# ishine/minimax-speech

Hardware: AMD Instinct MI355X
Metric: 24 kHz audio-seconds generated per wall-second per node (CosyVoice2-0.5B-shaped LM + flow + DAC-VAE, end to end) (higher is better)
Workload: dtype bf16

## Files before the change

### minimax-speech_amd/csrc/attention_x.hip

```cpp
#include "common.h"
#include "../../include/mmx_hip.h"
#include <cstdlib>
#include <type_traits>
#include <utility>

namespace {

__device__ __forceinline__ int swz(int row, int c) { return row * 128 + ((c ^ (row & 7)) << 4); }

__device__ __forceinline__ void split4(const float x[4], uint2& hi, uint2& lo) {
    hi.x = pack_bf16x2(x[0], x[1]);
    hi.y = pack_bf16x2(x[2], x[3]);
    lo.x = pack_bf16x2(x[0] - __uint_as_float(hi.x << 16), x[1] - __uint_as_float(hi.x & 0xffff0000u));
    lo.y = pack_bf16x2(x[2] - __uint_as_float(hi.y << 16), x[3] - __uint_as_float(hi.y & 0xffff0000u));
}

template <int MF, bool PRE, int NW>
__global__ __launch_bounds__(64 * NW) void attn_flash_x_kernel(
    const void* __restrict__ q_, long ldq, long q_bs, const void* __restrict__ k_, long ldk, long k_bs,
    const void* __restrict__ v_, long ldv, long v_bs, float* __restrict__ out, long ldo, long o_bs,
    int Tn, float scale, const float* __restrict__ keymask, long km_bs, int chunk, int nq, int nheads, int npairs,
    int q_begin, const int32_t* __restrict__ klen) {
    typedef std::conditional_t<PRE, bf16_t, float> TI;
    const TI* q = reinterpret_cast<const TI*>(q_);
    const TI* k = reinterpret_cast<const TI*>(k_);
    const TI* v = reinterpret_cast<const TI*>(v_);
    constexpr int D = 64, KT = 64, QW = 16 * MF;
    constexpr int TILE = KT * 128;
    extern __shared__ __attribute__((aligned(16))) char smem[];
    char* Kh = smem;
    char* Kl = Kh + 2 * TILE;
    char* Vh = Kl + 2 * TILE;
    char* Vl = Vh + 2 * TILE;
    char* Ph = Vl + 2 * TILE;
    char* Pl = Ph + NW * QW * 128;
    const int tid = threadIdx.x, lane = tid & 63, wave = tid >> 6;
    const int g = lane >> 4, l16 = lane & 15;
    const int xcd = blockIdx.x & 7, slot = blockIdx.x >> 3;
    const int pair = (slot / nq) * 8 + xcd;
    if (pair >= npairs) return;
    const int qt = slot % nq;
    const int b = pair / nheads, h = pair % nheads;
    const int qb = q_begin + qt * (NW * QW) + wave * QW;
    q += (long)b * q_bs + h * D;
    k += (long)b * k_bs + h * D;
    v += PRE ? (long)b * v_bs + (long)h * D * ldv : (long)b * v_bs + h * D;
    out += (long)b * o_bs + h * D;
    const float* km = keymask ? keymask + (long)b * km_bs : nullptr;
    const float sc2 = scale * 1.44269504088896341f;
    const int Tk = klen ? (klen[b] < Tn ? klen[b] : Tn) : Tn;
    if (klen && q_begin + qt * (NW * QW) >= Tk) {
        for (int id = tid; id < NW * QW * 16; id += 64 * NW) {
            const int i = q_begin + qt * (NW * QW) + (id >> 4);
            if (i < Tn) *reinterpret_cast<float4*>(out + (long)i * ldo + (id & 15) * 4) = make_float4(0.f, 0.f, 0.f, 0.f);
        }
        return;
    }

    short8_t aqh[MF][2], aql[MF][2];
#pragma unroll
    for (int mf = 0; mf < MF; ++mf) {
        int row = qb + mf * 16 + l16;
        row = row < Tn ? row : Tn - 1;
#pragma unroll
        for (int ks = 0; ks < 2; ++ks) {
            if constexpr (PRE) {
                const bf16_t* qp = reinterpret_cast<const bf16_t*>(q) + (long)row * ldq + ks * 32 + 8 * g;
                aqh[mf][ks] = *reinterpret_cast<const short8_t*>(qp);
                aql[mf][ks] = *reinterpret_cast<const short8_t*>(qp + 1024);
            } else {
                const float* qp = reinterpret_cast<const float*>(q) + (long)row * ldq + ks * 32 + 8 * g;
                const float4 a = *reinterpret_cast<const float4*>(qp), c = *reinterpret_cast<const float4*>(qp + 4);
                const float x0[4] = {a.x, a.y, a.z, a.w}, x1[4] = {c.x, c.y, c.z, c.w};
                uint2 h0, l0, h1, l1;
                split4(x0, h0, l0);
                split4(x1, h1, l1);
                aqh[mf][ks] = __builtin_bit_cast(short8_t, make_uint4(h0.x, h0.y, h1.x, h1.y));
                aql[mf][ks] = __builtin_bit_cast(short8_t, make_uint4(l0.x, l0.y, l1.x, l1.y));
            }
        }
    }
    float4_t o[MF][4];
    float m_run[MF], l_run[MF];
    int lim[MF];
#pragma unroll
    for (int mf = 0; mf < MF; ++mf) {
#pragma unroll
        for (int i = 0; i < 4; ++i) o[mf][i] = float4_t{0.f, 0.f, 0.f, 0.f};
        m_run[mf] = -INFINITY;
        l_run[mf] = 0.f;
        const int i = qb + mf * 16 + l16;
        int e = Tk;
        if (chunk > 0) { int c2 = (i / chunk + 1) * chunk; e = c2 < e ? c2 : e; }
        lim[mf] = e;
    }
    int kend = Tk;
    if (chunk > 0) {
        int qlast = q_begin + qt * (NW * QW) + NW * QW - 1;
        if (qlast > Tn - 1) qlast = Tn - 1;
        int e = (qlast / chunk + 1) * chunk;
        if (e < kend) kend = e;
    }
    const int ntile = (kend + KT - 1) / KT;
    int vis_all = Tk;
    if (chunk > 0) {
        const int e = ((q_begin + qt * (NW * QW)) / chunk + 1) * chunk;
        if (e < vis_all) vis_all = e;
    }
    char* Pwh = Ph + wave * QW * 128;
    char* Pwl = Pl + wave * QW * 128;

    constexpr int NT = 64 * NW, CPT = 1024 / NT;
    float4 kreg[CPT], vreg[CPT];
    auto load_tiles = [&](int j0) {
        if constexpr (PRE) {
            const bf16_t* kb = reinterpret_cast<const bf16_t*>(k);
            const bf16_t* vb = reinterpret_cast<const bf16_t*>(v);
#pragma unroll
            for (int pi = 0; pi < CPT / 2; ++pi) {
                const int id = tid + pi * NT, r = id >> 3, c = (id & 7) * 8;
                const int key = j0 + r;
#pragma unroll
                for (int pl = 0; pl < 2; ++pl) {
                    kreg[2 * pi + pl] = key < Tk ? *reinterpret_cast<const float4*>(kb + (long)key * ldk + pl * 1024 + c) : make_float4(0.f, 0.f, 0.f, 0.f);
                    vreg[2 * pi + pl] = (j0 + c < Tk) ? *reinterpret_cast<const float4*>(vb + (long)pl * 512 * ldv + (long)r * ldv + j0 + c) : make_float4(0.f, 0.f, 0.f, 0.f);
                }
            }
            return;
        }
#pragma unroll
        for (int i = 0; i < CPT; ++i) {
            const int id = tid + i * NT;
            const int kr = j0 + (id >> 4);
            kreg[i] = kr < Tk ? *reinterpret_cast<const float4*>(reinterpret_cast<const float*>(k) + (long)kr * ldk + (id & 15) * 4) : make_float4(0.f, 0.f, 0.f, 0.f);
            const int vr = j0 + 2 * (id >> 5) + (id & 1);
            vreg[i] = vr < Tk ? *reinterpret_cast<const float4*>(reinterpret_cast<const float*>(v) + (long)vr * ldv + ((id >> 1) & 15) * 4) : make_float4(0.f, 0.f, 0.f, 0.f);
        }
    };
    auto store_tiles = [&](int buf) {
        if constexpr (PRE) {
#pragma unroll
            for (int pi = 0; pi < CPT / 2; ++pi) {
                const int id = tid + pi * NT, r = id >> 3, c8 = id & 7;
                const int off = buf * TILE + swz(r, c8);
                *reinterpret_cast<float4*>(Kh + off) = kreg[2 * pi];
                *reinterpret_cast<float4*>(Kl + off) = kreg[2 * pi + 1];
                *reinterpret_cast<float4*>(Vh + off) = vreg[2 * pi];
                *reinterpret_cast<float4*>(Vl + off) = vreg[2 * pi + 1];
            }
            return;
        }
#pragma unroll
        for (int i = 0; i < CPT; ++i) {
            const int id = tid + i * NT;
            {
                const int r = id >> 4, c4 = id & 15;
                const float x[4] = {kreg[i].x, kreg[i].y, kreg[i].z, kreg[i].w};
                uint2 hi, lo;
                split4(x, hi, lo);
                const int off = buf * TILE + swz(r, c4 >> 1) + (c4 & 1) * 8;
                *reinterpret_cast<uint2*>(Kh + off) = hi;
                *reinterpret_cast<uint2*>(Kl + off) = lo;
            }
            {
                const int par = id & 1, cc = (id >> 1) & 15, kp = id >> 5;
                const float s0 = par ? vreg[i].x : vreg[i].z, s1 = par ? vreg[i].y : vreg[i].w;
                const float r0 = __shfl_xor(s0, 1, 64), r1 = __shfl_xor(s1, 1, 64);
                const float a0 = par ? r0 : vreg[i].x, b0 = par ? vreg[i].z : r0;
                const float a1 = par ? r1 : vreg[i].y, b1 = par ? vreg[i].w : r1;
                const int d0 = 4 * cc + 2 * par;
                const unsigned h0 = pack_bf16x2(a0, b0), h1 = pack_bf16x2(a1, b1);
                const unsigned l0 = pack_bf16x2(a0 - __uint_as_float(h0 << 16), b0 - __uint_as_float(h0 & 0xffff0000u));
                const unsigned l1 = pack_bf16x2(a1 - __uint_as_float(h1 << 16), b1 - __uint_as_float(h1 & 0xffff0000u));
                const int o0 = buf * TILE + swz(d0, kp >> 2) + (kp & 3) * 4, o1 = buf * TILE + swz(d0 + 1, kp >> 2) + (kp & 3) * 4;
                *reinterpret_cast<unsigned*>(Vh + o0) = h0;
                *reinterpret_cast<unsigned*>(Vl + o0) = l0;
                *reinterpret_cast<unsigned*>(Vh + o1) = h1;
                *reinterpret_cast<unsigned*>(Vl + o1) = l1;
            }
        }
    };
    load_tiles(0);
    store_tiles(0);
    if (ntile > 1) load_tiles(KT);
    for (int jt = 0; jt < ntile; ++jt) {
        const int j0 = jt * KT, buf = jt & 1;
        __syncthreads();
        if (jt + 1 < ntile) store_tiles(buf ^ 1);
        if (jt + 2 < ntile) load_tiles(j0 + 2 * KT);
        float4_t s[MF][4];
#pragma unroll
        for (int nf = 0; nf < 4; ++nf) {
#pragma unroll
            for (int mf = 0; mf < MF; ++mf) s[mf][nf] = float4_t{0.f, 0.f, 0.f, 0.f};
#pragma unroll
            for (int ks = 0; ks < 2; ++ks) {
                const int off = buf * TILE + swz(nf * 16 + l16, ks * 4 + g);
                const short8_t bkh = *reinterpret_cast<const short8_t*>(Kh + off);
                const short8_t bkl = *reinterpret_cast<const short8_t*>(Kl + off);
#pragma unroll
                for (int mf = 0; mf < MF; ++mf) {
                    s[mf][nf] = __builtin_amdgcn_mfma_f32_16x16x32_bf16(bkh, aqh[mf][ks], s[mf][nf], 0, 0, 0);
                    s[mf][nf] = __builtin_amdgcn_mfma_f32_16x16x32_bf16(bkh, aql[mf][ks], s[mf][nf], 0, 0, 0);
                    s[mf][nf] = __builtin_amdgcn_mfma_f32_16x16x32_bf16(bkl, aqh[mf][ks], s[mf][nf], 0, 0, 0);
                }
            }
        }
        const bool need_mask = km || (j0 + KT > vis_all);
        bool kvis[4][4];
        if (need_mask) {
#pragma unroll
            for (int nf = 0; nf < 4; ++nf)
#pragma unroll
                for (int r = 0; r < 4; ++r) {
                    const int j = j0 + nf * 16 + 4 * g + r;
                    kvis[nf][r] = j < Tk && (!km || km[j] != 0.f);
                }
        }
        auto softmax_tile = [&](auto mask_c, auto mf_c) {
            constexpr bool MASK = decltype(mask_c)::value;
            constexpr int mf = decltype(mf_c)::value;
            float mx = -INFINITY;
#pragma unroll
            for (int nf = 0; nf < 4; ++nf)
#pragma unroll
                for (int r = 0; r < 4; ++r) {
                    float x = s[mf][nf][r];
                    if constexpr (MASK) {
                        const int j = j0 + nf * 16 + 4 * g + r;
                        x = (j < lim[mf] && kvis[nf][r]) ? x : -INFINITY;
                        s[mf][nf][r] = x;
                    }
                    mx = fmaxf(mx, x);
                }
            mx *= sc2;
            float m_use = m_run[mf];
            const bool grow = (mx - m_run[mf]) > 6.0f || m_run[mf] == -INFINITY;
            if (__any(grow)) {
                mx = fmaxf(mx, __shfl_xor(mx, 16, 64));
                mx = fmaxf(mx, __shfl_xor(mx, 32, 64));
                const float m_new = fmaxf(m_run[mf], mx);
                const float m_safe = m_new == -INFINITY ? 0.f : m_new;
                const float alpha = __builtin_amdgcn_exp2f(m_run[mf] - m_safe);
                l_run[mf] *= alpha;
#pragma unroll
                for (int df = 0; df < 4; ++df)
#pragma unroll
                    for (int r = 0; r < 4; ++r) o[mf][df][r] *= alpha;
                m_run[mf] = m_new;
                m_use = m_safe;
            }
            float rs = 0.f;
#pragma unroll
            for (int nf = 0; nf < 4; ++nf) {
                float p[4];
#pragma unroll
                for (int r = 0; r < 4; ++r) p[r] = __builtin_amdgcn_exp2f(__builtin_fmaf(s[mf][nf][r], sc2, -m_use));
                rs += (p[0] + p[1]) + (p[2] + p[3]);
                uint2 hi, lo;
                split4(p, hi, lo);
                const int off = swz(mf * 16 + l16, nf * 2 + (g >> 1)) + (g & 1) * 8;
                *reinterpret_cast<uint2*>(Pwh + off) = hi;
                *reinterpret_cast<uint2*>(Pwl + off) = lo;
            }
            l_run[mf] += rs;
        };
        if (need_mask) {
            softmax_tile(std::true_type{}, std::integral_constant<int, 0>{});
            if constexpr (MF > 1) softmax_tile(std::true_type{}, std::integral_constant<int, MF - 1>{});
        } else {
            softmax_tile(std::false_type{}, std::integral_constant<int, 0>{});
            if constexpr (MF > 1) softmax_tile(std::false_type{}, std::integral_constant<int, MF - 1>{});
        }
        __builtin_amdgcn_fence(__ATOMIC_RELEASE, "wavefront");
        __builtin_amdgcn_wave_barrier();
        short8_t aph[MF][2], apl[MF][2];
#pragma unroll
        for (int mf = 0; mf < MF; ++mf)
#pragma unroll
            for (int ks = 0; ks < 2; ++ks) {
                const int off = swz(mf * 16 + l16, ks * 4 + g);
                aph[mf][ks] = *reinterpret_cast<const short8_t*>(Pwh + off);
                apl[mf][ks] = *reinterpret_cast<const short8_t*>(Pwl + off);
            }
#pragma unroll
        for (int df = 0; df < 4; ++df)
#pragma unroll
            for (int ks = 0; ks < 2; ++ks) {
                const int off = buf * TILE + swz(df * 16 + l16, ks * 4 + g);
                const short8_t bvh = *reinterpret_cast<const short8_t*>(Vh + off);
                const short8_t bvl = *reinterpret_cast<const short8_t*>(Vl + off);
#pragma unroll
                for (int mf = 0; mf < MF; ++mf) {
                    o[mf][df] = __builtin_amdgcn_mfma_f32_16x16x32_bf16(bvh, aph[mf][ks], o[mf][df], 0, 0, 0);
                    o[mf][df] = __builtin_amdgcn_mfma_f32_16x16x32_bf16(bvh, apl[mf][ks], o[mf][df], 0, 0, 0);
                    o[mf][df] = __builtin_amdgcn_mfma_f32_16x16x32_bf16(bvl, aph[mf][ks], o[mf][df], 0, 0, 0);
                }
            }
        __builtin_amdgcn_wave_barrier();
    }
#pragma unroll
    for (int mf = 0; mf < MF; ++mf) {
        l_run[mf] += __shfl_xor(l_run[mf], 16, 64);
        l_run[mf] += __shfl_xor(l_run[mf], 32, 64);
    }
#pragma unroll
    for (int mf = 0; mf < MF; ++mf) {
        const int i = qb + mf * 16 + l16;
        if (i >= Tn) continue;
        const float inv = l_run[mf] > 0.f ? 1.f / l_run[mf] : 0.f;
#pragma unroll
        for (int df = 0; df < 4; ++df)
            *reinterpret_cast<float4*>(out + (long)i * ldo + df * 16 + 4 * g) =
                make_float4(o[mf][df][0] * inv, o[mf][df][1] * inv, o[mf][df][2] * inv, o[mf][df][3] * inv);
    }
}

__global__ __launch_bounds__(256) void attn_relpos_x_kernel(
    const float* __restrict__ q, long ldq, long q_bs, const float* __restrict__ k, long ldk, long k_bs,
    const float* __restrict__ v, long ldv, long v_bs, const float* __restrict__ pos, long ldp,
    const float* __restrict__ pos_u, const float* __restrict__ pos_v, float* __restrict__ out, long ldo, long o_bs,
    int Tn, float scale, int chunk, int nq, int nheads, int npairs, const int32_t* __restrict__ klen) {
    constexpr int D = 64, KT = 64, NW = 4, QW = 16, BW = 84;
    constexpr int TILE = KT * 128;
    extern __shared__ __attribute__((aligned(16))) char smem[];
    char* Kh = smem;
    char* Kl = Kh + 2 * TILE;
    char* Vh = Kl + 2 * TILE;
    char* Vl = Vh + 2 * TILE;
    char* Ph = Vl + 2 * TILE;
    char* Pl = Ph + NW * QW * 128;
    float* Bp = reinterpret_cast<float*>(Pl + NW * QW * 128);
    const int tid = threadIdx.x, lane = tid & 63, wave = tid >> 6;
    const int g = lane >> 4, l16 = lane & 15;
    const int xcd = blockIdx.x & 7, slot = blockIdx.x >> 3;
    const int pair = (slot / nq) * 8 + xcd;
    if (pair >= npairs) return;
    const int qt = slot % nq;
    const int b = pair / nheads, h = pair % nheads;
    const int qb = qt * (NW * QW) + wave * QW;
    q += (long)b * q_bs + h * D;
    k += (long)b * k_bs + h * D;
    v += (long)b * v_bs + h * D;
    out += (long)b * o_bs + h * D;
    pos += h * D;
    const float sc2 = scale * 1.44269504088896341f;
    const int Tk = klen ? (klen[b] < Tn ? klen[b] : Tn) : Tn;

    short8_t auh[2], aul[2], avh[2], avl[2];
    {
        int row = qb + l16;
        row = row < Tn ? row : Tn - 1;
#pragma unroll
        for (int ks = 0; ks < 2; ++ks) {
            const float* qp = q + (long)row * ldq + ks * 32 + 8 * g;
            const float4 a = *reinterpret_cast<const float4*>(qp), c = *reinterpret_cast<const float4*>(qp + 4);
            const float* pu = pos_u + h * D + ks * 32 + 8 * g;
            const float* pv = pos_v + h * D + ks * 32 + 8 * g;
            const float x[8] = {a.x, a.y, a.z, a.w, c.x, c.y, c.z, c.w};
            float xu0[4], xu1[4], xv0[4], xv1[4];
#pragma unroll
            for (int e = 0; e < 4; ++e) {
                xu0[e] = x[e] + pu[e]; xu1[e] = x[4 + e] + pu[4 + e];
                xv0[e] = x[e] + pv[e]; xv1[e] = x[4 + e] + pv[4 + e];
            }
            uint2 h0, l0, h1, l1;
            split4(xu0, h0, l0);
            split4(xu1, h1, l1);
            auh[ks] = __builtin_bit_cast(short8_t, make_uint4(h0.x, h0.y, h1.x, h1.y));
            aul[ks] = __builtin_bit_cast(short8_t, make_uint4(l0.x, l0.y, l1.x, l1.y));
            split4(xv0, h0, l0);
            split4(xv1, h1, l1);
            avh[ks] = __builtin_bit_cast(short8_t, make_uint4(h0.x, h0.y, h1.x, h1.y));
            avl[ks] = __builtin_bit_cast(short8_t, make_uint4(l0.x, l0.y, l1.x, l1.y));
        }
    }
    float4_t o[4];
#pragma unroll
    for (int i = 0; i < 4; ++i) o[i] = float4_t{0.f, 0.f, 0.f, 0.f};
    float m_run = -INFINITY, l_run = 0.f;
    int lim = Tk;
    if (chunk > 0) { const int c2 = ((qb + l16) / chunk + 1) * chunk; lim = c2 < lim ? c2 : lim; }
    int kend = Tk;
    if (chunk > 0) {
        int qlast = qt * (NW * QW) + NW * QW - 1;
        if (qlast > Tn - 1) qlast = Tn - 1;
        const int e = (qlast / chunk + 1) * chunk;
        if (e < kend) kend = e;
    }
    const int ntile = (kend + KT - 1) / KT;
    int vis_all = Tk;
    if (chunk > 0) {
        const int e = ((qt * (NW * QW)) / chunk + 1) * chunk;
        if (e < vis_all) vis_all = e;
    }
    char* Pwh = Ph + wave * QW * 128;
    char* Pwl = Pl + wave * QW * 128;
    float* Bw = Bp + wave * 16 * BW;

    constexpr int NT = 64 * NW, CPT = 1024 / NT;
    float4 kreg[CPT], vreg[CPT];
    auto load_tiles = [&](int j0) {
#pragma unroll
        for (int i = 0; i < CPT; ++i) {
            const int id = tid + i * NT;
            const int kr = j0 + (id >> 4);
            kreg[i] = kr < Tk ? *reinterpret_cast<const float4*>(k + (long)kr * ldk + (id & 15) * 4) : make_float4(0.f, 0.f, 0.f, 0.f);
            const int vr = j0 + 2 * (id >> 5) + (id & 1);
            vreg[i] = vr < Tk ? *reinterpret_cast<const float4*>(v + (long)vr * ldv + ((id >> 1) & 15) * 4) : make_float4(0.f, 0.f, 0.f, 0.f);
        }
    };
    auto store_tiles = [&](int buf) {
#pragma unroll
        for (int i = 0; i < CPT; ++i) {
            const int id = tid + i * NT;
            {
                const int r = id >> 4, c4 = id & 15;
                const float x[4] = {kreg[i].x, kreg[i].y, kreg[i].z, kreg[i].w};
                uint2 hi, lo;
                split4(x, hi, lo);
                const int off = buf * TILE + swz(r, c4 >> 1) + (c4 & 1) * 8;
                *reinterpret_cast<uint2*>(Kh + off) = hi;
                *reinterpret_cast<uint2*>(Kl + off) = lo;
            }
            {
                const int par = id & 1, cc = (id >> 1) & 15, kp = id >> 5;
                const float s0 = par ? vreg[i].x : vreg[i].z, s1 = par ? vreg[i].y : vreg[i].w;
                const float r0 = __shfl_xor(s0, 1, 64), r1 = __shfl_xor(s1, 1, 64);
                const float a0 = par ? r0 : vreg[i].x, b0 = par ? vreg[i].z : r0;
                const float a1 = par ? r1 : vreg[i].y, b1 = par ? vreg[i].w : r1;
                const int d0 = 4 * cc + 2 * par;
                const unsigned h0 = pack_bf16x2(a0, b0), h1 = pack_bf16x2(a1, b1);
                const unsigned l0 = pack_bf16x2(a0 - __uint_as_float(h0 << 16), b0 - __uint_as_float(h0 & 0xffff0000u));
                const unsigned l1 = pack_bf16x2(a1 - __uint_as_float(h1 << 16), b1 - __uint_as_float(h1 & 0xffff0000u));
                const int o0 = buf * TILE + swz(d0, kp >> 2) + (kp & 3) * 4, o1 = buf * TILE + swz(d0 + 1, kp >> 2) + (kp & 3) * 4;
                *reinterpret_cast<unsigned*>(Vh + o0) = h0;
                *reinterpret_cast<unsigned*>(Vl + o0) = l0;
                *reinterpret_cast<unsigned*>(Vh + o1) = h1;
                *reinterpret_cast<unsigned*>(Vl + o1) = l1;
            }
        }
    };
    float4 praw[5][2][2];
    const int prow_max = 2 * Tn - 2;
    auto load_window = [&](int j0) {
        const int mbase = Tn - 1 - (qb + 15) + j0;
#pragma unroll
        for (int f = 0; f < 5; ++f) {
            int row = mbase + f * 16 + l16;
            row = row < 0 ? 0 : (row > prow_max ? prow_max : row);
            const float* pp = pos + (long)row * ldp + 8 * g;
#pragma unroll
            for (int ks = 0; ks < 2; ++ks) {
                praw[f][ks][0] = *reinterpret_cast<const float4*>(pp + ks * 32);
                praw[f][ks][1] = *reinterpret_cast<const float4*>(pp + ks * 32 + 4);
            }
        }
    };
    load_tiles(0);
    store_tiles(0);
    if (ntile > 1) load_tiles(KT);
    load_window(0);
    for (int jt = 0; jt < ntile; ++jt) {
        const int j0 = jt * KT, buf = jt & 1;
        __syncthreads();
        if (jt + 1 < ntile) store_tiles(buf ^ 1);
        if (jt + 2 < ntile) load_tiles(j0 + 2 * KT);
        float4_t bd[5];
#pragma unroll
        for (int f = 0; f < 5; ++f) {
            bd[f] = float4_t{0.f, 0.f, 0.f, 0.f};
#pragma unroll
            for (int ks = 0; ks < 2; ++ks) {
                const float x0[4] = {praw[f][ks][0].x, praw[f][ks][0].y, praw[f][ks][0].z, praw[f][ks][0].w};
                const float x1[4] = {praw[f][ks][1].x, praw[f][ks][1].y, praw[f][ks][1].z, praw[f][ks][1].w};
                uint2 h0, l0, h1, l1;
                split4(x0, h0, l0);
                split4(x1, h1, l1);
                const short8_t ph = __builtin_bit_cast(short8_t, make_uint4(h0.x, h0.y, h1.x, h1.y));
                const short8_t pl = __builtin_bit_cast(short8_t, make_uint4(l0.x, l0.y, l1.x, l1.y));
                bd[f] = __builtin_amdgcn_mfma_f32_16x16x32_bf16(ph, avh[ks], bd[f], 0, 0, 0);
                bd[f] = __builtin_amdgcn_mfma_f32_16x16x32_bf16(ph, avl[ks], bd[f], 0, 0, 0);
                bd[f] = __builtin_amdgcn_mfma_f32_16x16x32_bf16(pl, avh[ks], bd[f], 0, 0, 0);
            }
        }
        if (jt + 1 < ntile) load_window(j0 + KT);
#pragma unroll
        for (int f = 0; f < 5; ++f) *reinterpret_cast<float4_t*>(Bw + l16 * BW + f * 16 + 4 * g) = bd[f];
        float4_t s[4];
#pragma unroll
        for (int nf = 0; nf < 4; ++nf) {
            s[nf] = float4_t{0.f, 0.f, 0.f, 0.f};
#pragma unroll
            for (int ks = 0; ks < 2; ++ks) {
                const int off = buf * TILE + swz(nf * 16 + l16, ks * 4 + g);
                const short8_t bkh = *reinterpret_cast<const short8_t*>(Kh + off);
                const short8_t bkl = *reinterpret_cast<const short8_t*>(Kl + off);
                s[nf] = __builtin_amdgcn_mfma_f32_16x16x32_bf16(bkh, auh[ks], s[nf], 0, 0, 0);
                s[nf] = __builtin_amdgcn_mfma_f32_16x16x32_bf16(bkh, aul[ks], s[nf], 0, 0, 0);
                s[nf] = __builtin_amdgcn_mfma_f32_16x16x32_bf16(bkl, auh[ks], s[nf], 0, 0, 0);
            }
        }
        __builtin_amdgcn_fence(__ATOMIC_RELEASE, "wavefront");
        __builtin_amdgcn_wave_barrier();
        {
            const float* src = Bw + l16 * BW + 15 - l16 + 4 * g;
#pragma unroll
            for (int nf = 0; nf < 4; ++nf)
#pragma unroll
                for (int r = 0; r < 4; ++r) s[nf][r] += src[nf * 16 + r];
        }
        __builtin_amdgcn_fence(__ATOMIC_RELEASE, "wavefront");
        __builtin_amdgcn_wave_barrier();
        const bool need_mask = j0 + KT > vis_all;
        float mx = -INFINITY;
#pragma unroll
        for (int nf = 0; nf < 4; ++nf)
#pragma unroll
            for (int r = 0; r < 4; ++r) {
                float x = s[nf][r];
                if (need_mask) {
                    const int j = j0 + nf * 16 + 4 * g + r;
                    x = j < lim ? x : -INFINITY;
                    s[nf][r] = x;
                }
                mx = fmaxf(mx, x);
            }
        mx *= sc2;
        float m_use = m_run;
        const bool grow = (mx - m_run) > 6.0f || m_run == -INFINITY;
        if (__any(grow)) {
            mx = fmaxf(mx, __shfl_xor(mx, 16, 64));
            mx = fmaxf(mx, __shfl_xor(mx, 32, 64));
            const float m_new = fmaxf(m_run, mx);
            const float m_safe = m_new == -INFINITY ? 0.f : m_new;
            const float alpha = __builtin_amdgcn_exp2f(m_run - m_safe);
            l_run *= alpha;
#pragma unroll
            for (int df = 0; df < 4; ++df)
#pragma unroll
                for (int r = 0; r < 4; ++r) o[df][r] *= alpha;
            m_run = m_new;
            m_use = m_safe;
        }
        float rs = 0.f;
#pragma unroll
        for (int nf = 0; nf < 4; ++nf) {
            float p[4];
#pragma unroll
            for (int r = 0; r < 4; ++r) p[r] = __builtin_amdgcn_exp2f(__builtin_fmaf(s[nf][r], sc2, -m_use));
            rs += (p[0] + p[1]) + (p[2] + p[3]);
            uint2 hi, lo;
            split4(p, hi, lo);
            const int off = swz(l16, nf * 2 + (g >> 1)) + (g & 1) * 8;
            *reinterpret_cast<uint2*>(Pwh + off) = hi;
            *reinterpret_cast<uint2*>(Pwl + off) = lo;
        }
        l_run += rs;
        __builtin_amdgcn_fence(__ATOMIC_RELEASE, "wavefront");
        __builtin_amdgcn_wave_barrier();
        short8_t aph[2], apl[2];
#pragma unroll
        for (int ks = 0; ks < 2; ++ks) {
            const int off = swz(l16, ks * 4 + g);
            aph[ks] = *reinterpret_cast<const short8_t*>(Pwh + off);
            apl[ks] = *reinterpret_cast<const short8_t*>(Pwl + off);
        }
#pragma unroll
        for (int df = 0; df < 4; ++df)
#pragma unroll
            for (int ks = 0; ks < 2; ++ks) {
                const int off = buf * TILE + swz(df * 16 + l16, ks * 4 + g);
                const short8_t bvh = *reinterpret_cast<const short8_t*>(Vh + off);
                const short8_t bvl = *reinterpret_cast<const short8_t*>(Vl + off);
                o[df] = __builtin_amdgcn_mfma_f32_16x16x32_bf16(bvh, aph[ks], o[df], 0, 0, 0);
                o[df] = __builtin_amdgcn_mfma_f32_16x16x32_bf16(bvh, apl[ks], o[df], 0, 0, 0);
                o[df] = __builtin_amdgcn_mfma_f32_16x16x32_bf16(bvl, aph[ks], o[df], 0, 0, 0);
            }
        __builtin_amdgcn_wave_barrier();
    }
    l_run += __shfl_xor(l_run, 16, 64);
    l_run += __shfl_xor(l_run, 32, 64);
    const int i = qb + l16;
    if (i < Tn) {
        const float inv = l_run > 0.f ? 1.f / l_run : 0.f;
#pragma unroll
        for (int df = 0; df < 4; ++df)
            *reinterpret_cast<float4*>(out + (long)i * ldo + df * 16 + 4 * g) = make_float4(o[df][0] * inv, o[df][1] * inv, o[df][2] * inv, o[df][3] * inv);
    }
}

template <int MF, bool PRE, int NW>
int launch_flash_x(dim3 grid, hipStream_t stream, const void* q, long ldq, long q_bs, const void* k, long ldk, long k_bs,
                   const void* v, long ldv, long v_bs, float* out, long ldo, long o_bs, int T_, float scale,
                   const float* keymask, long km_bs, int chunk, int nq, int H, int npairs, int q_begin, const int32_t* klen) {
    const size_t lds = (size_t)8 * 64 * 128 + (size_t)2 * NW * 16 * MF * 128;
    MMX_LDS_OPT_IN((attn_flash_x_kernel<MF, PRE, NW>), lds);
    hipLaunchKernelGGL((attn_flash_x_kernel<MF, PRE, NW>), grid, dim3(64 * NW), lds, stream, q, ldq, q_bs, k, ldk, k_bs, v, ldv, v_bs, out, ldo, o_bs, T_,
                       scale, keymask, km_bs, chunk, nq, H, npairs, q_begin, klen);
    MMX_LAUNCH_CHECK();
    return MMX_OK;
}

}

extern "C" int mmx_attn_flash_x(const float* q, int64_t ldq, int64_t q_bs, const float* k, int64_t ldk, int64_t k_bs,
                                const float* v, int64_t ldv, int64_t v_bs, float* out, int64_t ldo, int64_t o_bs,
                                int B, int H, int T_, float scale, const float* keymask, int64_t km_bs, int chunk,
                                int q_begin, const int32_t* klen, hipStream_t stream) {
    MMX_CHECK_ARG(q && k && v && out && B > 0 && H > 0 && T_ > 0 && chunk >= 0);
    MMX_CHECK_ARG(q_begin >= 0 && q_begin < T_ && q_begin % 16 == 0);
    MMX_CHECK_ARG(ldq % 4 == 0 && ldk % 4 == 0 && ldv % 4 == 0 && ldo % 4 == 0 && q_bs % 4 == 0 && k_bs % 4 == 0 && v_bs % 4 == 0 && o_bs % 4 == 0);
    MMX_CHECK_ARG(((uintptr_t)q % 16) == 0 && ((uintptr_t)k % 16) == 0 && ((uintptr_t)v % 16) == 0 && ((uintptr_t)out % 16) == 0);
    const int npairs = H * B, Tq = T_ - q_begin;
    const bool small = (long)npairs * ((Tq + 127) / 128) < 192;
    const int qtile = small ? 64 : 128, nq = (Tq + qtile - 1) / qtile;
    dim3 grid(8 * ((npairs + 7) / 8) * nq);
    if (small) return launch_flash_x<1, false, 4>(grid, stream, q, ldq, q_bs, k, ldk, k_bs, v, ldv, v_bs, out, ldo, o_bs, T_, scale, keymask, km_bs, chunk, nq, H, npairs, q_begin, klen);
    return launch_flash_x<1, false, 8>(grid, stream, q, ldq, q_bs, k, ldk, k_bs, v, ldv, v_bs, out, ldo, o_bs, T_, scale, keymask, km_bs, chunk, nq, H, npairs, q_begin, klen);
}

extern "C" int mmx_attn_flash_xs(const void* qk, int64_t ldqk, int64_t qk_bs, const void* vt, int64_t ldvt, int64_t vt_bs,
                                 float* out, int64_t ldo, int64_t o_bs, int B, int H, int T_, float scale, const float* keymask,
                                 int64_t km_bs, int chunk, int q_begin, const int32_t* klen, int form, hipStream_t stream) {
    MMX_CHECK_ARG(qk && vt && out && B > 0 && H > 0 && H * 64 <= 512 && T_ > 0 && chunk >= 0 && form >= 0 && form <= 3);
    MMX_CHECK_ARG(q_begin >= 0 && q_begin < T_ && q_begin % 16 == 0);
    MMX_CHECK_ARG(ldqk >= 2048 && ldqk % 8 == 0 && qk_bs % 8 == 0 && ldvt % 8 == 0 && ldvt >= ((T_ + 7) / 8) * 8 && vt_bs % 8 == 0 && vt_bs >= 2 * 512 * ldvt);
    MMX_CHECK_ARG(ldo % 4 == 0 && o_bs % 4 == 0 && ((uintptr_t)qk % 16) == 0 && ((uintptr_t)vt % 16) == 0 && ((uintptr_t)out % 16) == 0);
    const int npairs = H * B, Tq = T_ - q_begin;
    const bool small = form == 3 || (long)npairs * ((Tq + 127) / 128) < 192;
    const int qtile = small ? 64 : 128, nq = (Tq + qtile - 1) / qtile;
    dim3 grid(8 * ((npairs + 7) / 8) * nq);
    const bf16_t* q = (const bf16_t*)qk;
    const int nq2 = (Tq + 255) / 256;
    const long wg1 = (long)npairs * nq, wg2 = (long)npairs * nq2;
    const bool mf2 = !small && form != 1 && (form == 2 || 1.6 * (double)((wg2 + 255) / 256) < (double)((wg1 + 255) / 256));
    if (mf2) {
        dim3 grid2(8 * ((npairs + 7) / 8) * nq2);
        return launch_flash_x<2, true, 8>(grid2, stream, q, ldqk, qk_bs, q + 512, ldqk, qk_bs, vt, ldvt, vt_bs, out, ldo, o_bs, T_, scale, keymask, km_bs, chunk, nq2, H, npairs, q_begin, klen);
    }
    if (small) return launch_flash_x<1, true, 4>(grid, stream, q, ldqk, qk_bs, q + 512, ldqk, qk_bs, vt, ldvt, vt_bs, out, ldo, o_bs, T_, scale, keymask, km_bs, chunk, nq, H, npairs, q_begin, klen);
    return launch_flash_x<1, true, 8>(grid, stream, q, ldqk, qk_bs, q + 512, ldqk, qk_bs, vt, ldvt, vt_bs, out, ldo, o_bs, T_, scale, keymask, km_bs, chunk, nq, H, npairs, q_begin, klen);
}

extern "C" int mmx_attn_relpos_x(const float* q, int64_t ldq, int64_t q_bs, const float* k, int64_t ldk, int64_t k_bs,
                                 const float* v, int64_t ldv, int64_t v_bs, const float* pos, int64_t ldp, const float* pos_u,
                                 const float* pos_v, float* out, int64_t ldo, int64_t o_bs, int B, int H, int T_, float scale,
                                 int chunk, const int32_t* klen, hipStream_t stream) {
    MMX_CHECK_ARG(q && k && v && pos && pos_u && pos_v && out && B > 0 && H > 0 && T_ > 0 && chunk >= 0);
    MMX_CHECK_ARG(ldq % 4 == 0 && ldk % 4 == 0 && ldv % 4 == 0 && ldp % 4 == 0 && ldo % 4 == 0 && q_bs % 4 == 0 && k_bs % 4 == 0 && v_bs % 4 == 0 && o_bs % 4 == 0);
    MMX_CHECK_ARG(((uintptr_t)q % 16) == 0 && ((uintptr_t)k % 16) == 0 && ((uintptr_t)v % 16) == 0 && ((uintptr_t)pos % 16) == 0 &&
                  ((uintptr_t)out % 16) == 0 && ((uintptr_t)pos_u % 16) == 0 && ((uintptr_t)pos_v % 16) == 0);
    const int npairs = H * B, nq = (T_ + 63) / 64;
    const size_t lds = (size_t)8 * 64 * 128 + (size_t)2 * 4 * 16 * 128 + (size_t)4 * 16 * 84 * 4;
    MMX_LDS_OPT_IN(attn_relpos_x_kernel, lds);
    hipLaunchKernelGGL(attn_relpos_x_kernel, dim3(8 * ((npairs + 7) / 8) * nq), dim3(256), lds, stream, q, ldq, q_bs, k, ldk, k_bs, v, ldv, v_bs,
                       pos, ldp, pos_u, pos_v, out, ldo, o_bs, T_, scale, chunk, nq, H, npairs, klen);
    MMX_LAUNCH_CHECK();
    return MMX_OK;
}
```

Measured before the change: 549.7.

## Keep softmax P in registers by permuting K rows, dropping LDS round-trip

K tile rows are stored in a permuted order (krow), so the S accumulator layout from the QK MFMA lines up with the A-operand layout needed by the PV MFMA. Softmax probabilities can then be packed straight into registers instead of being written to and read back from per-wave LDS. This removes the P staging buffers, their wave barriers and fence, and shrinks LDS per block. It also caps VGPRs for the 1/true/8 kernel variant and restricts the MF=2 path to explicit form==2, which changes the kernel chosen under default heuristics.

```diff
diff --git a/minimax-speech_amd/csrc/attention_x.hip b/minimax-speech_amd/csrc/attention_x.hip
--- a/minimax-speech_amd/csrc/attention_x.hip
+++ b/minimax-speech_amd/csrc/attention_x.hip
@@ -8,6 +8,8 @@
 
 __device__ __forceinline__ int swz(int row, int c) { return row * 128 + ((c ^ (row & 7)) << 4); }
 
+__device__ __forceinline__ int krow(int key) { return (key & 32) | ((key & 4) << 2) | ((key >> 1) & 12) | (key & 3); }
+
 __device__ __forceinline__ void split4(const float x[4], uint2& hi, uint2& lo) {
     hi.x = pack_bf16x2(x[0], x[1]);
     hi.y = pack_bf16x2(x[2], x[3]);
@@ -16,7 +18,7 @@
 }
 
 template <int MF, bool PRE, int NW>
-__global__ __launch_bounds__(64 * NW) void attn_flash_x_kernel(
+__device__ __forceinline__ void attn_flash_x_body(
     const void* __restrict__ q_, long ldq, long q_bs, const void* __restrict__ k_, long ldk, long k_bs,
     const void* __restrict__ v_, long ldv, long v_bs, float* __restrict__ out, long ldo, long o_bs,
     int Tn, float scale, const float* __restrict__ keymask, long km_bs, int chunk, int nq, int nheads, int npairs,
@@ -32,8 +34,6 @@
     char* Kl = Kh + 2 * TILE;
     char* Vh = Kl + 2 * TILE;
     char* Vl = Vh + 2 * TILE;
-    char* Ph = Vl + 2 * TILE;
-    char* Pl = Ph + NW * QW * 128;
     const int tid = threadIdx.x, lane = tid & 63, wave = tid >> 6;
     const int g = lane >> 4, l16 = lane & 15;
     const int xcd = blockIdx.x & 7, slot = blockIdx.x >> 3;
@@ -107,8 +107,6 @@
         const int e = ((q_begin + qt * (NW * QW)) / chunk + 1) * chunk;
         if (e < vis_all) vis_all = e;
     }
-    char* Pwh = Ph + wave * QW * 128;
-    char* Pwl = Pl + wave * QW * 128;
 
     constexpr int NT = 64 * NW, CPT = 1024 / NT;
     float4 kreg[CPT], vreg[CPT];
@@ -142,9 +140,9 @@
 #pragma unroll
             for (int pi = 0; pi < CPT / 2; ++pi) {
                 const int id = tid + pi * NT, r = id >> 3, c8 = id & 7;
-                const int off = buf * TILE + swz(r, c8);
-                *reinterpret_cast<float4*>(Kh + off) = kreg[2 * pi];
-                *reinterpret_cast<float4*>(Kl + off) = kreg[2 * pi + 1];
+                const int koff = buf * TILE + swz(krow(r), c8), off = buf * TILE + swz(r, c8);
+                *reinterpret_cast<float4*>(Kh + koff) = kreg[2 * pi];
+                *reinterpret_cast<float4*>(Kl + koff) = kreg[2 * pi + 1];
                 *reinterpret_cast<float4*>(Vh + off) = vreg[2 * pi];
                 *reinterpret_cast<float4*>(Vl + off) = vreg[2 * pi + 1];
             }
@@ -154,7 +152,7 @@
         for (int i = 0; i < CPT; ++i) {
             const int id = tid + i * NT;
             {
-                const int r = id >> 4, c4 = id & 15;
+                const int r = krow(id >> 4), c4 = id & 15;
                 const float x[4] = {kreg[i].x, kreg[i].y, kreg[i].z, kreg[i].w};
                 uint2 hi, lo;
                 split4(x, hi, lo);
@@ -213,10 +211,11 @@
             for (int nf = 0; nf < 4; ++nf)
 #pragma unroll
                 for (int r = 0; r < 4; ++r) {
-                    const int j = j0 + nf * 16 + 4 * g + r;
+                    const int j = j0 + (nf >> 1) * 32 + 8 * g + (nf & 1) * 4 + r;
                     kvis[nf][r] = j < Tk && (!km || km[j] != 0.f);
                 }
         }
+        short8_t aph[MF][2], apl[MF][2];
         auto softmax_tile = [&](auto mask_c, auto mf_c) {
             constexpr bool MASK = decltype(mask_c)::value;
             constexpr int mf = decltype(mf_c)::value;
@@ -227,7 +226,7 @@
                 for (int r = 0; r < 4; ++r) {
                     float x = s[mf][nf][r];
                     if constexpr (MASK) {
-                        const int j = j0 + nf * 16 + 4 * g + r;
+                        const int j = j0 + (nf >> 1) * 32 + 8 * g + (nf & 1) * 4 + r;
                         x = (j < lim[mf] && kvis[nf][r]) ? x : -INFINITY;
                         s[mf][nf][r] = x;
                     }
@@ -251,19 +250,21 @@
                 m_use = m_safe;
             }
             float rs = 0.f;
+            uint2 hi[4], lo[4];
 #pragma unroll
             for (int nf = 0; nf < 4; ++nf) {
                 float p[4];
 #pragma unroll
                 for (int r = 0; r < 4; ++r) p[r] = __builtin_amdgcn_exp2f(__builtin_fmaf(s[mf][nf][r], sc2, -m_use));
                 rs += (p[0] + p[1]) + (p[2] + p[3]);
-                uint2 hi, lo;
-                split4(p, hi, lo);
-                const int off = swz(mf * 16 + l16, nf * 2 + (g >> 1)) + (g & 1) * 8;
-                *reinterpret_cast<uint2*>(Pwh + off) = hi;
-                *reinterpret_cast<uint2*>(Pwl + off) = lo;
+                split4(p, hi[nf], lo[nf]);
             }
             l_run[mf] += rs;
+#pragma unroll
+            for (int ks = 0; ks < 2; ++ks) {
+                aph[mf][ks] = __builtin_bit_cast(short8_t, make_uint4(hi[2 * ks].x, hi[2 * ks].y, hi[2 * ks + 1].x, hi[2 * ks + 1].y));
+                apl[mf][ks] = __builtin_bit_cast(short8_t, make_uint4(lo[2 * ks].x, lo[2 * ks].y, lo[2 * ks + 1].x, lo[2 * ks + 1].y));
+            }
         };
         if (need_mask) {
             softmax_tile(std::true_type{}, std::integral_constant<int, 0>{});
@@ -272,17 +273,6 @@
             softmax_tile(std::false_type{}, std::integral_constant<int, 0>{});
             if constexpr (MF > 1) softmax_tile(std::false_type{}, std::integral_constant<int, MF - 1>{});
         }
-        __builtin_amdgcn_fence(__ATOMIC_RELEASE, "wavefront");
-        __builtin_amdgcn_wave_barrier();
-        short8_t aph[MF][2], apl[MF][2];
-#pragma unroll
-        for (int mf = 0; mf < MF; ++mf)
-#pragma unroll
-            for (int ks = 0; ks < 2; ++ks) {
-                const int off = swz(mf * 16 + l16, ks * 4 + g);
-                aph[mf][ks] = *reinterpret_cast<const short8_t*>(Pwh + off);
-                apl[mf][ks] = *reinterpret_cast<const short8_t*>(Pwl + off);
-            }
 #pragma unroll
         for (int df = 0; df < 4; ++df)
 #pragma unroll
@@ -297,7 +287,6 @@
                     o[mf][df] = __builtin_amdgcn_mfma_f32_16x16x32_bf16(bvl, aph[mf][ks], o[mf][df], 0, 0, 0);
                 }
             }
-        __builtin_amdgcn_wave_barrier();
     }
 #pragma unroll
     for (int mf = 0; mf < MF; ++mf) {
@@ -314,6 +303,21 @@
             *reinterpret_cast<float4*>(out + (long)i * ldo + df * 16 + 4 * g) =
                 make_float4(o[mf][df][0] * inv, o[mf][df][1] * inv, o[mf][df][2] * inv, o[mf][df][3] * inv);
     }
+}
+
+#define MMX_FLASH_X_PARAMS                                                                                                      \
+    const void *__restrict__ q, long ldq, long q_bs, const void *__restrict__ k, long ldk, long k_bs, const void *__restrict__ v, \
+        long ldv, long v_bs, float *__restrict__ out, long ldo, long o_bs, int Tn, float scale, const float *__restrict__ keymask, \
+        long km_bs, int chunk, int nq, int nheads, int npairs, int q_begin, const int32_t *__restrict__ klen
+#define MMX_FLASH_X_ARGS q, ldq, q_bs, k, ldk, k_bs, v, ldv, v_bs, out, ldo, o_bs, Tn, scale, keymask, km_bs, chunk, nq, nheads, npairs, q_begin, klen
+
+template <int MF, bool PRE, int NW>
+__global__ __launch_bounds__(64 * NW) void attn_flash_x_kernel(MMX_FLASH_X_PARAMS) {
+    attn_flash_x_body<MF, PRE, NW>(MMX_FLASH_X_ARGS);
+}
+template <>
+__global__ __launch_bounds__(512) __attribute__((amdgpu_num_vgpr(136))) void attn_flash_x_kernel<1, true, 8>(MMX_FLASH_X_PARAMS) {
+    attn_flash_x_body<1, true, 8>(MMX_FLASH_X_ARGS);
 }
 
 __global__ __launch_bounds__(256) void attn_relpos_x_kernel(
@@ -594,7 +598,7 @@
 int launch_flash_x(dim3 grid, hipStream_t stream, const void* q, long ldq, long q_bs, const void* k, long ldk, long k_bs,
                    const void* v, long ldv, long v_bs, float* out, long ldo, long o_bs, int T_, float scale,
                    const float* keymask, long km_bs, int chunk, int nq, int H, int npairs, int q_begin, const int32_t* klen) {
-    const size_t lds = (size_t)8 * 64 * 128 + (size_t)2 * NW * 16 * MF * 128;
+    const size_t lds = (size_t)8 * 64 * 128;
     MMX_LDS_OPT_IN((attn_flash_x_kernel<MF, PRE, NW>), lds);
     hipLaunchKernelGGL((attn_flash_x_kernel<MF, PRE, NW>), grid, dim3(64 * NW), lds, stream, q, ldq, q_bs, k, ldk, k_bs, v, ldv, v_bs, out, ldo, o_bs, T_,
                        scale, keymask, km_bs, chunk, nq, H, npairs, q_begin, klen);
@@ -633,8 +637,7 @@
     dim3 grid(8 * ((npairs + 7) / 8) * nq);
     const bf16_t* q = (const bf16_t*)qk;
     const int nq2 = (Tq + 255) / 256;
-    const long wg1 = (long)npairs * nq, wg2 = (long)npairs * nq2;
-    const bool mf2 = !small && form != 1 && (form == 2 || 1.6 * (double)((wg2 + 255) / 256) < (double)((wg1 + 255) / 256));
+    const bool mf2 = !small && form == 2;
     if (mf2) {
         dim3 grid2(8 * ((npairs + 7) / 8) * nq2);
         return launch_flash_x<2, true, 8>(grid2, stream, q, ldqk, qk_bs, q + 512, ldqk, qk_bs, vt, ldvt, vt_bs, out, ldo, o_bs, T_, scale, keymask, km_bs, chunk, nq2, H, npairs, q_begin, klen);
```

Measured after the change: 556.7 (median of 6 runs). 1.3% higher.
